# HKUST-Aerial-Robotics/FUEL

Measured on AMD Instinct MI355X. Metric: plan_cycles_per_sec, higher is better.
Workload: dtype u64 bit-planes / u16 (u32 beyond 255 voxels) exact squared distances / f32 ESDF / f64 log-odds and B-spline

## Files before the change

### fuel_amd/csrc/bspline.hip

```cpp
#include <cmath>
#include <cstring>
#include <vector>

#include "bspline_batch.h"

template <int CTRL, int ROW_MASK>
__device__ __forceinline__ double dpp_take(double v) {
  int lo = __double2loint(v), hi = __double2hiint(v);
  lo = __builtin_amdgcn_update_dpp(0, lo, CTRL, ROW_MASK, 0xF, false);
  hi = __builtin_amdgcn_update_dpp(0, hi, CTRL, ROW_MASK, 0xF, false);
  return __hiloint2double(hi, lo);
}
__device__ __forceinline__ double wave_sum(double v) {
  v += dpp_take<0xB1, 0xF>(v);
  v += dpp_take<0x4E, 0xF>(v);
  v += dpp_take<0x141, 0xF>(v);
  v += dpp_take<0x140, 0xF>(v);
  v += dpp_take<0x142, 0xA>(v);
  v += dpp_take<0x143, 0xC>(v);
  const int lo = __builtin_amdgcn_readlane(__double2loint(v), 63), hi = __builtin_amdgcn_readlane(__double2hiint(v), 63);
  return __hiloint2double(hi, lo);
}

__device__ __forceinline__ double dot3(const double* a, const double* b) {
  return a[0] * b[0] + a[1] * b[1] + a[2] * b[2];
}

#define EVAL_CONST 24
__device__ __forceinline__ double* eval_const(const BsplineArgs& A, unsigned char* smem_raw) {
  return reinterpret_cast<double*>(smem_raw) + 15 * (size_t)A.N;
}
__device__ void load_eval_const(const BsplineArgs& A, int c, unsigned char* smem_raw) {
  double* K = eval_const(A, smem_raw);
  const int l = threadIdx.x;
  if (l == 0) K[0] = A.pt_dist[c];
  if (l == 1) K[1] = A.knot_span ? A.knot_span[c] : 0.0;
  if (l == 2) K[2] = A.time_lb ? A.time_lb[c] : -1.0;
  if (l >= 3 && l < 12) K[l] = ((A.cost_function & FUELMI_COST_START) && A.start_state) ? A.start_state[(size_t)c * 9 + (l - 3)] : 0.0;
  if (l >= 12 && l < 21) K[l] = ((A.cost_function & FUELMI_COST_END) && A.end_state) ? A.end_state[(size_t)c * 9 + (l - 12)] : 0.0;
  __syncthreads();
}
template <int NWV>
__device__ double bspline_eval(const Geo& g, const float* __restrict__ dist, const BsplineArgs& A, int c,
                               const double* x, double* grad, unsigned char* smem_raw) {
  const double* K = eval_const(A, smem_raw);
  const int N = A.N, dim = A.dim;
  const int wv = NWV == 1 ? 0 : (int)(threadIdx.x >> 6);
  const bool is_sm = NWV == 1 || wv == 0, is_fe = NWV == 1 || wv == 1, is_di = NWV == 1 || wv == 2, is_mi = NWV == 1 || wv == 3;
  double* q = reinterpret_cast<double*>(smem_raw);
  double* tj = q + 3 * N;
  double* tv = tj + 3 * N;
  double* ta = tv + 3 * N;
  double* gw = ta + 3 * N;
  const int lane = threadIdx.x & 63;
  const bool opt_time = (A.cost_function & FUELMI_COST_MINTIME) != 0;
  const double dt = opt_time ? x[A.nvar - 1] : K[1];
  const double pt_dist = K[0];
  const fuelmi_bspline_cfg& P = A.cfg;

  for (int i = threadIdx.x; i < N; i += 64 * NWV)
    for (int j = 0; j < 3; ++j) q[3 * i + j] = (j < dim) ? x[dim * i + j] : 0.0;
  __syncthreads();

  double cost = 0.0, gt = 0.0;
  const double dt_inv = 1 / dt, dt_inv2 = dt_inv * dt_inv;
  const double pt_inv = 1 / pt_dist;
  const double r_2dt = 1 / (2 * dt), r_dt2 = 1 / (dt * dt), r_ndt2 = 1 / (-dt * dt), r_ndt3 = 1 / (-dt * dt * dt);
  DistGather G0;
  const bool gather0 = is_di && (A.cost_function & FUELMI_COST_DISTANCE) && lane < N;
  if (gather0) dist_gather_issue(g, dist, &q[3 * lane], G0);

  for (int i = lane; i < N; i += 64) {
    for (int k = 0; k < 3; ++k) {
      if (is_sm) tj[3 * i + k] = 0.0;
      if (is_fe) tv[3 * i + k] = 0.0;
      if (is_fe) ta[3 * i + k] = 0.0;
      if (is_mi) gw[3 * i + k] = 0.0;
    }
    if (is_sm && (A.cost_function & FUELMI_COST_SMOOTHNESS) && i + 3 < N) {
      double s = 0.0;
      for (int k = 0; k < 3; ++k) {
        double ji = (q[3 * (i + 3) + k] - 3 * q[3 * (i + 2) + k] + 3 * q[3 * (i + 1) + k] - q[3 * i + k]) * pt_inv;
        s += ji * ji;
        tj[3 * i + k] = 2 * ji * pt_inv;
      }
      cost += P.ld_smooth * s;
    }
    if (is_fe && (A.cost_function & FUELMI_COST_FEASIBILITY)) {
      if (i + 1 < N) {
        for (int k = 0; k < 3; ++k) {
          double vi = (q[3 * (i + 1) + k] - q[3 * i + k]) * dt_inv;
          double vd = fabs(vi) - P.max_vel;
          if (vd > 0.0) {
            cost += P.ld_feasi * (vd * vd);
            double sign = vi > 0 ? 1.0 : -1.0;
            double tmp = 2 * vd * sign * dt_inv;
            tv[3 * i + k] = tmp;
            if (opt_time) gt += P.ld_feasi * (tmp * (-vi));
          }
        }
      }
      if (i + 2 < N) {
        for (int k = 0; k < 3; ++k) {
          double ai = (q[3 * (i + 2) + k] - 2 * q[3 * (i + 1) + k] + q[3 * i + k]) * dt_inv2;
          double ad = fabs(ai) - P.max_acc;
          if (ad > 0.0) {
            cost += P.ld_feasi * (ad * ad);
            double sign = ai > 0 ? 1.0 : -1.0;
            double tmp = 2 * ad * sign * dt_inv2;
            ta[3 * i + k] = tmp;
            if (opt_time) gt += P.ld_feasi * (tmp * ai * (-2) * dt);
          }
        }
      }
    }
  }
  __syncthreads();
  if (is_mi && (A.cost_function & FUELMI_COST_WAYPOINTS) && lane == 0) {
    double s = 0.0;
    for (int w = 0; w < A.n_waypt; ++w) {
      const double* wp = A.waypoints + ((size_t)c * A.n_waypt + w) * 3;
      int idx = A.waypt_idx[(size_t)c * A.n_waypt + w];
      for (int k = 0; k < 3; ++k) {
        double dq = 1 / 6.0 * (q[3 * idx + k] + 4 * q[3 * (idx + 1) + k] + q[3 * (idx + 2) + k]) - wp[k];
        s += dq * dq;
        gw[3 * idx + k] += dq * (2.0 / 6.0);
        gw[3 * (idx + 1) + k] += dq * (8.0 / 6.0);
        gw[3 * (idx + 2) + k] += dq * (2.0 / 6.0);
      }
    }
    cost += P.ld_waypt * s;
  }
  __syncthreads();

  for (int i = lane; i < N; i += 64) {
    double gq[3] = {0.0, 0.0, 0.0};
    if (is_sm && (A.cost_function & FUELMI_COST_SMOOTHNESS)) {
      const double wgt[4] = {-1.0, 3.0, -3.0, 1.0};
      for (int s = 0; s < 4; ++s) {
        int j = i - s;
        if (j >= 0 && j + 3 < N)
          for (int k = 0; k < 3; ++k) gq[k] += P.ld_smooth * wgt[s] * tj[3 * j + k];
      }
    }
    if (is_di && (A.cost_function & FUELMI_COST_DISTANCE)) {
      double dg[3];
      double d = (i == lane && gather0) ? dist_gather_finish(g, G0, dg) : dist_with_grad_dev(g, dist, &q[3 * i], dg);
      double nrm = sqrt(dot3(dg, dg));
      if (nrm > 1e-4) {
        const double nrm_inv = 1 / nrm;
        for (int k = 0; k < 3; ++k) dg[k] *= nrm_inv;
      }
      if (d < P.dist0) {
        cost += P.ld_dist * ((d - P.dist0) * (d - P.dist0));
        for (int k = 0; k < 3; ++k) gq[k] += P.ld_dist * (2.0 * (d - P.dist0) * dg[k]);
      }
    }
    if (is_fe && (A.cost_function & FUELMI_COST_FEASIBILITY)) {
      for (int k = 0; k < 3; ++k) {
        double s = 0.0;
        if (i + 1 < N) s += -tv[3 * i + k];
        if (i >= 1) s += tv[3 * (i - 1) + k];
        if (i + 2 < N) s += ta[3 * i + k];
        if (i >= 1 && i + 1 < N) s += -2 * ta[3 * (i - 1) + k];
        if (i >= 2) s += ta[3 * (i - 2) + k];
        gq[k] += P.ld_feasi * s;
      }
    }
    {
      const bool is_start = is_mi && (A.cost_function & FUELMI_COST_START) && i < 3;
      const bool is_end = is_mi && (A.cost_function & FUELMI_COST_END) && i >= N - 3;
      for (int pass = 0; pass < 2; ++pass) {
        const bool as_end = (pass == 0) ? (!is_start && is_end) : (is_start && is_end);
        if (!(pass == 0 ? (is_start || is_end) : as_end)) continue;
        const int b0 = as_end ? N - 3 : 0, r = i - b0;
        const double* tgt = K + (as_end ? 12 : 3);
        const double w_pos = as_end ? 1.0 : 10.0, lam = as_end ? P.ld_end : P.ld_start;
        const bool have_vel = !as_end || A.end_n >= 2, have_acc = !as_end || A.end_n == 3;
        double c_b = 0.0, gt_b = 0.0;
        for (int k = 0; k < 3; ++k) {
          const double qa = q[3 * b0 + k], qb = q[3 * (b0 + 1) + k], qc = q[3 * (b0 + 2) + k];
          const double first = as_end ? qc : qa, last = as_end ? qa : qc;
          double dq = 1 / 6.0 * (first + 4 * qb + last) - tgt[k];
          c_b += w_pos * dq * dq;
          double gk = w_pos * 2 * dq * ((r == 1) ? (4 / 6.0) : (1 / 6.0));
          if (have_vel) {
            dq = r_2dt * (qc - qa) - tgt[3 + k];
            c_b += dq * dq;
            if (r == 0) gk += 2 * dq * (-1.0) * r_2dt;
            if (r == 2) gk += 2 * dq * 1.0 * r_2dt;
            gt_b += dq * (qc - qa) * r_ndt2;
          }
          if (have_acc) {
            dq = r_dt2 * (first - 2 * qb + last) - tgt[6 + k];
            c_b += dq * dq;
            gk += 2 * dq * ((r == 1) ? -2.0 : 1.0) * r_dt2;
            gt_b += dq * (first - 2 * qb + last) * r_ndt3;
          }
          gq[k] += lam * gk;
        }
        if (r == (as_end ? 2 : 0)) {
          cost += lam * c_b;
          if (opt_time) gt += lam * gt_b;
        }
      }
    }
    if (is_mi && (A.cost_function & FUELMI_COST_GUIDE) && i >= A.order && i < N - A.order) {
      const double* gp = A.guide_pts + ((size_t)c * A.n_guide + (i - A.order)) * 3;
      for (int k = 0; k < 3; ++k) {
        double d = q[3 * i + k] - gp[k];
        cost += P.ld_guide * d * d;
        gq[k] += P.ld_guide * 2 * d;
      }
    }
    if (is_mi && (A.cost_function & FUELMI_COST_WAYPOINTS))
      for (int k = 0; k < 3; ++k) gq[k] += P.ld_waypt * gw[3 * i + k];
    if (is_mi && (A.cost_function & FUELMI_COST_VIEWCONS) && i == A.view_idx[c]) {
      const double* p = A.view_pt + (size_t)c * 3;
      const double* dir = A.view_dir + (size_t)c * 3;
      double dn_ = sqrt(dot3(dir, dir));
      double v[3] = {dir[0] / dn_, dir[1] / dn_, dir[2] / dn_};
      double qp[3] = {q[3 * i] - p[0], q[3 * i + 1] - p[1], q[3 * i + 2] - p[2]};
      double pr = dot3(qp, v);
      double dn[3], dl[3];
      for (int k = 0; k < 3; ++k) {
        dn[k] = qp[k] - pr * v[k];
        dl[k] = pr * v[k];
      }
      double c_view = dot3(dn, dn);
      double vdn = dot3(v, dn);
      for (int k = 0; k < 3; ++k) gq[k] += P.ld_view * 2 * (dn[k] - vdn * v[k]);
      double norm_dl = sqrt(dot3(dl, dl));
      if (norm_dl < dn_) {
        c_view += P.wnl * (norm_dl - dn_) * (norm_dl - dn_);
        double vdl = dot3(v, dl);
        for (int k = 0; k < 3; ++k) gq[k] += P.ld_view * (P.wnl * 2 * (norm_dl - dn_) * (vdl * v[k]) / norm_dl);
      }
      cost += P.ld_view * c_view;
    }
    if (NWV == 1) {
      for (int j = 0; j < dim; ++j) grad[dim * i + j] = gq[j];
    } else {
      double* gpart = reinterpret_cast<double*>(smem_raw) + 15 * (size_t)N + EVAL_CONST + (size_t)wv * 3 * N;
      for (int j = 0; j < 3; ++j) gpart[3 * i + j] = gq[j];
    }
  }

  if (is_mi && (A.cost_function & FUELMI_COST_MINTIME) && lane == 0) {
    double duration = (N - A.order) * dt;
    double cst = duration, g_t = double(N - A.order);
    double lb = K[2];
    if (lb > 0 && duration < lb) {
      const double w_lb = 10;
      cst += w_lb * (duration - lb) * (duration - lb);
      g_t += w_lb * 2 * (duration - lb) * (N - A.order);
    }
    cost += P.ld_time * cst;
    gt += P.ld_time * g_t;
  }
  cost = wave_sum(cost);
  gt = wave_sum(gt);
  if (NWV == 1) {
    if (lane == 0 && opt_time) grad[A.nvar - 1] = gt;
    __syncthreads();
    return cost;
  }
  double* part = reinterpret_cast<double*>(smem_raw) + 15 * (size_t)N + EVAL_CONST;
  double* cpart = part + 12 * (size_t)N;
  if (lane == 0) cpart[wv] = cost, cpart[4 + wv] = gt;
  __syncthreads();
  for (int e = threadIdx.x; e < dim * N; e += 64 * NWV) {
    const int i = e / dim, j = e - i * dim;
    grad[e] = ((part[3 * i + j] + part[3 * N + 3 * i + j]) + part[6 * N + 3 * i + j]) + part[9 * N + 3 * i + j];
  }
  if (threadIdx.x == 0 && opt_time) grad[A.nvar - 1] = ((cpart[4] + cpart[5]) + cpart[6]) + cpart[7];
  const double total = ((cpart[0] + cpart[1]) + cpart[2]) + cpart[3];
  __syncthreads();
  return total;
}

__global__ void __launch_bounds__(256)
k_bspline_cost_grad(Geo g, const float* __restrict__ dist, BsplineArgs A) {
  extern __shared__ __attribute__((aligned(16))) unsigned char smem_raw[];
  const int c = blockIdx.x;
  load_eval_const(A, c, smem_raw);
  const double cost = bspline_eval<4>(g, dist, A, c, A.x + (size_t)c * A.nvar, A.grad + (size_t)c * A.nvar, smem_raw);
  if (threadIdx.x == 0) A.cost[c] = cost;
}

struct LbfgsArgs {
  int max_eval;
  unsigned long long max_ticks;
  double box_lo[3], box_hi[3];
  double* x_out;
  double* cost_out;
  int* evals_out;
};
#define LBFGS_MEM 8

__device__ __forceinline__ double wdot(const double* a, const double* b, int n) {
  double s = 0.0;
  for (int i = threadIdx.x; i < n; i += 64) s += a[i] * b[i];
  return wave_sum(s);
}

__global__ void __launch_bounds__(64)
k_bspline_optimize(Geo g, const float* __restrict__ dist, BsplineArgs A, LbfgsArgs L) {
  extern __shared__ __attribute__((aligned(16))) unsigned char smem_raw[];
  const int c = blockIdx.x, lane = threadIdx.x, n = A.nvar;
  double* w = reinterpret_cast<double*>(smem_raw) + 15 * (size_t)A.N + EVAL_CONST;
  load_eval_const(A, blockIdx.x, smem_raw);
  double *q = w, *gq = q + n, *xn = gq + n, *gn = xn + n, *d = gn + n, *best = d + n;
  double* S = best + n;
  double* Y = S + LBFGS_MEM * n;
  double* rho = Y + LBFGS_MEM * n;
  double* al = rho + LBFGS_MEM;
  const double* x0 = A.x + (size_t)c * n;
  const int npt = A.dim * A.N;
  auto lb_of = [&](int i, double q0) {
    if (A.dim == 1) return -1e300;
    if (i >= npt) return 0.0;
    return fmax(q0 - 10.0, L.box_lo[i % 3]);
  };
  auto ub_of = [&](int i, double q0) {
    if (A.dim == 1) return 1e300;
    if (i >= npt) return 5.0;
    return fmin(q0 + 10.0, L.box_hi[i % 3]);
  };
  for (int i = lane; i < n; i += 64) {
    double v = x0[i];
    if (A.dim != 1 && i < npt) v = fmax(fmin(v, L.box_hi[i % 3]), L.box_lo[i % 3]);
    q[i] = v;
    best[i] = v;
  }
  __syncthreads();
  auto start_val = [&](int i) {
    double v = x0[i];
    if (A.dim != 1 && i < npt) v = fmax(fmin(v, L.box_hi[i % 3]), L.box_lo[i % 3]);
    return v;
  };
  int evals = 0;
  const unsigned long long t_begin = wall_clock64();
  auto out_of_time = [&]() { return L.max_ticks != 0ull && wall_clock64() - t_begin > L.max_ticks; };
  double f = bspline_eval<1>(g, dist, A, c, q, gq, smem_raw);
  ++evals;
  double fbest = f;
  int hist = 0, head = 0;
  while (evals < L.max_eval && !out_of_time()) {
    for (int i = lane; i < n; i += 64) {
      const double sv = start_val(i), lo = lb_of(i, sv), hi = ub_of(i, sv);
      const bool at_lb = q[i] <= lo && gq[i] > 0, at_ub = q[i] >= hi && gq[i] < 0;
      d[i] = (at_lb || at_ub) ? 0.0 : -gq[i];
    }
    __syncthreads();
    for (int k = hist - 1; k >= 0; --k) {
      const int sl = (head + k) % LBFGS_MEM;
      const double a = wdot(S + sl * n, d, n) * rho[sl];
      if (lane == 0) al[sl] = a;
      for (int i = lane; i < n; i += 64) d[i] -= a * Y[sl * n + i];
      __syncthreads();
    }
    if (hist > 0) {
      const int sl = (head + hist - 1) % LBFGS_MEM;
      const double yy = wdot(Y + sl * n, Y + sl * n, n), sy = 1.0 / rho[sl];
      const double gamma = yy > 0 ? sy / yy : 1.0;
      for (int i = lane; i < n; i += 64) d[i] *= gamma;
      __syncthreads();
    }
    for (int k = 0; k < hist; ++k) {
      const int sl = (head + k) % LBFGS_MEM;
// ... 414 lines not shown
    }
    F.pt_dist[c] = s / double(n);
  }
}
static size_t fit_lds(int K, int degree) {
  const int n = K + degree - 1;
  return (size_t)(16 + 5 * n + 3 * n + 3 * n + 3 * (K + 4) + n + degree + 1) * sizeof(double);
}

__global__ __launch_bounds__(64) void k_bspline_boundary(int n, int p, const double* __restrict__ ts,
                                                         const double* __restrict__ ctrl, int ks, int ke,
                                                         double* __restrict__ start, double* __restrict__ end) {
  extern __shared__ __attribute__((aligned(16))) unsigned char smem_raw[];
  double* q = reinterpret_cast<double*>(smem_raw);
  double* u = q + 3 * n;
  const int c = blockIdx.x, lane = threadIdx.x;
  for (int i = lane; i < 3 * n; i += 64) q[i] = ctrl[(size_t)c * 3 * n + i];
  if (lane == 0) fit_uniform_knots(u, n, p, ts[c]);
  __syncthreads();
  if (lane <= ks) spline_boundary_value(q, n, p, u, lane, false, start + ((size_t)c * (ks + 1) + lane) * 3);
  else if (lane <= ks + 1 + ke)
    spline_boundary_value(q, n, p, u, lane - ks - 1, true, end + ((size_t)c * (ke + 1) + (lane - ks - 1)) * 3);
}

static int upload(fuelmi_bspline_dev* b, const void* src, size_t bytes, const void** dst) {
  *dst = nullptr;
  if (!src || bytes == 0) return FUELMI_OK;
  void* d = nullptr;
  HIPCHK(hipMalloc(&d, bytes));
  b->allocs.push_back(d);
  HIPCHK(hipMemcpyAsync(d, src, bytes, hipMemcpyHostToDevice, b->map->stream));
  *dst = d;
  return FUELMI_OK;
}

static void bspline_dev_orphan(void* p) { static_cast<fuelmi_bspline_dev*>(p)->map = nullptr; }
extern "C" void fuelmi_bspline_dev_destroy(fuelmi_bspline_dev* b) {
  if (!b) return;
  (void)hipSetDevice(b->device);
  if (b->map) {
    (void)hipStreamSynchronize(b->map->stream);
    std::lock_guard<std::mutex> lk(b->map->dep_mu);
    auto& deps = b->map->dependents;
    for (size_t k = 0; k < deps.size(); ++k)
      if (deps[k].obj == b) {
        deps.erase(deps.begin() + (long)k);
        break;
      }
  }
  for (void* p : b->allocs) (void)hipFree(p);
  for (DevScratch* sc : {&b->fit_in, &b->yaw_dev, &b->chk_dev, &b->smp_dev, &b->adj_dev}) sc->release();
  for (int k = 0; k < 2; ++k) {
    if (b->pin_out[k]) (void)hipHostFree(b->pin_out[k]);
    if (b->ev_out[k]) (void)hipEventDestroy(b->ev_out[k]);
  }
  delete b;
}

static int bspline_args_init(const fuelmi_bspline_cfg* cfg, const fuelmi_bspline_batch* in, BsplineArgs& A) {
  ARGCHK(in->dim >= 1 && in->dim <= 3 && in->point_num >= 4 && in->n_traj >= 1);
  ARGCHK(in->x && in->pt_dist);
  const int cf = in->cost_function;
  const bool opt_time = (cf & FUELMI_COST_MINTIME) != 0;
  ARGCHK(opt_time || in->knot_span);
  ARGCHK(!(cf & FUELMI_COST_START) || in->start_state);
  ARGCHK(!(cf & FUELMI_COST_END) || (in->end_state && in->end_n >= 1 && in->end_n <= 3));
  ARGCHK(!(cf & FUELMI_COST_GUIDE) || in->guide_pts);
  ARGCHK(!(cf & FUELMI_COST_WAYPOINTS) || (in->n_waypt >= 0 && (in->n_waypt == 0 || (in->waypoints && in->waypt_idx))));
  ARGCHK(!(cf & FUELMI_COST_VIEWCONS) || (in->view_pt && in->view_dir && in->view_idx));
  memset(&A, 0, sizeof(A));
  A.cfg = *cfg;
  A.cost_function = cf;
  A.dim = in->dim;
  A.N = in->point_num;
  A.C = in->n_traj;
  A.end_n = in->end_n;
  A.n_waypt = (cf & FUELMI_COST_WAYPOINTS) ? in->n_waypt : 0;
  A.nvar = opt_time ? A.dim * A.N + 1 : A.dim * A.N;
  A.order = (A.dim == 1) ? 3 : cfg->bspline_degree;
  A.n_guide = A.N - 2 * A.order;
  return FUELMI_OK;
}

extern "C" int fuelmi_bspline_dev_create(fuelmi_map* m, const fuelmi_bspline_cfg* cfg,
                                         const fuelmi_bspline_batch* in, fuelmi_bspline_dev** out) {
  ARGCHK(m && cfg && in && out);
  *out = nullptr;
  BsplineArgs A0;
  {
    const int rca = bspline_args_init(cfg, in, A0);
    if (rca) return rca;
  }
  const int cf = in->cost_function;
  const bool opt_time = (cf & FUELMI_COST_MINTIME) != 0;
  HIPCHK(hipSetDevice(m->device));
  fuelmi_bspline_dev* b = new fuelmi_bspline_dev;
  b->map = m;
  b->device = m->device;
  BsplineArgs& A = b->a;
  A = A0;
  (void)opt_time;
  b->lds = ((size_t)A.N * 3 * 5 + EVAL_CONST) * sizeof(double);
  b->lds_eval4 = b->lds + ((size_t)A.N * 12 + 8) * sizeof(double);
  if (b->lds_eval4 > 160 * 1024) {
    fuelmi_set_error("%d control points exceed the LDS budget", A.N);
    delete b;
    return FUELMI_ELIMIT;
  }
  const size_t C = (size_t)A.C;
  int rc = FUELMI_OK;
  auto up = [&](const void* src, size_t bytes, const void** dst) {
    if (rc == FUELMI_OK) rc = upload(b, src, bytes, dst);
  };
  up(in->x, C * A.nvar * sizeof(double), (const void**)&A.x);
  up(in->pt_dist, C * sizeof(double), (const void**)&A.pt_dist);
  up(in->knot_span, C * sizeof(double), (const void**)&A.knot_span);
  up(in->time_lb, C * sizeof(double), (const void**)&A.time_lb);
  if (cf & FUELMI_COST_START) up(in->start_state, C * 9 * sizeof(double), (const void**)&A.start_state);
  if (cf & FUELMI_COST_END) up(in->end_state, C * 9 * sizeof(double), (const void**)&A.end_state);
  if ((cf & FUELMI_COST_GUIDE) && A.n_guide > 0)
    up(in->guide_pts, C * A.n_guide * 3 * sizeof(double), (const void**)&A.guide_pts);
  if (A.n_waypt > 0) {
    up(in->waypoints, C * A.n_waypt * 3 * sizeof(double), (const void**)&A.waypoints);
    up(in->waypt_idx, C * A.n_waypt * sizeof(int), (const void**)&A.waypt_idx);
  }
  if (cf & FUELMI_COST_VIEWCONS) {
    up(in->view_pt, C * 3 * sizeof(double), (const void**)&A.view_pt);
    up(in->view_dir, C * 3 * sizeof(double), (const void**)&A.view_dir);
    up(in->view_idx, C * sizeof(int), (const void**)&A.view_idx);
  }
  if (rc == FUELMI_OK) {
    void* d = nullptr;
    if (hipMalloc(&d, C * sizeof(double)) == hipSuccess) {
      b->allocs.push_back(d);
      A.cost = (double*)d;
    } else
      rc = FUELMI_ENOMEM;
    if (rc == FUELMI_OK && hipMalloc(&d, C * A.nvar * sizeof(double)) == hipSuccess) {
      b->allocs.push_back(d);
      A.grad = (double*)d;
    } else
      rc = FUELMI_ENOMEM;
  }
  if (rc != FUELMI_OK) {
    fuelmi_bspline_dev_destroy(b);
    return rc;
  }
  if (b->lds_eval4 > 64 * 1024) {
    HIPCHK(hipFuncSetAttribute(reinterpret_cast<const void*>(&k_bspline_cost_grad),
                               hipFuncAttributeMaxDynamicSharedMemorySize, 160 * 1024));
  }
  {
    std::lock_guard<std::mutex> lk(m->dep_mu);
    m->dependents.push_back({b, &bspline_dev_orphan});
  }
  *out = b;
  return FUELMI_OK;
}

extern "C" int fuelmi_bspline_dev_eval(fuelmi_bspline_dev* b) {
  ARGCHK(b);
  HIPCHK(hipSetDevice(b->map->device));
  StageScope sc(b->map, FUELMI_K_BSPLINE);
  k_bspline_cost_grad<<<b->a.C, 256, b->lds_eval4, b->map->stream>>>(b->map->g, b->map->dist, b->a);
  HIPCHK(hipGetLastError());
  return FUELMI_OK;
}

extern "C" int fuelmi_bspline_dev_eval_pinned(fuelmi_bspline_dev* b, int slot) {
  ARGCHK(b && (slot == 0 || slot == 1));
  HIPCHK(hipSetDevice(b->map->device));
  const size_t C = (size_t)b->a.C, n = (size_t)b->a.nvar;
  if (!b->pin_out[slot]) {
    HIPCHK(hipHostMalloc(reinterpret_cast<void**>(&b->pin_out[slot]), (C + C * n) * sizeof(double), hipHostMallocDefault));
    HIPCHK(hipEventCreateWithFlags(&b->ev_out[slot], hipEventDisableTiming));
  }
  BsplineArgs A = b->a;
  A.cost = b->pin_out[slot];
  A.grad = b->pin_out[slot] + C;
  {
    StageScope sc(b->map, FUELMI_K_BSPLINE);
    k_bspline_cost_grad<<<A.C, 256, b->lds_eval4, b->map->stream>>>(b->map->g, b->map->dist, A);
    HIPCHK(hipGetLastError());
  }
  HIPCHK(hipEventRecord(b->ev_out[slot], b->map->stream));
  return FUELMI_OK;
}
extern "C" int fuelmi_bspline_dev_collect(fuelmi_bspline_dev* b, int slot, double* cost, double* grad) {
  ARGCHK(b && (slot == 0 || slot == 1) && cost && grad && b->pin_out[slot]);
  HIPCHK(hipSetDevice(b->map->device));
  HIPCHK(event_poll(b->ev_out[slot]));
  const size_t C = (size_t)b->a.C, n = (size_t)b->a.nvar;
  memcpy(cost, b->pin_out[slot], C * sizeof(double));
  memcpy(grad, b->pin_out[slot] + C, C * n * sizeof(double));
  return FUELMI_OK;
}

struct OptPlan {
  int npl, waves;
  size_t lds;
};
static int bspline_opt_plan(const BsplineArgs& A, OptPlan& p) {
  if (A.dim == 2) {
    fuelmi_set_error("the B-spline optimiser takes dim 1 or 3, not 2");
    return FUELMI_EINVAL;
  }
  const size_t n = (size_t)A.nvar;
  const size_t lds_eval = ((size_t)A.N * 3 * 5 + EVAL_CONST) * sizeof(double);
  p.npl = n <= 128 ? 2 : (n <= 256 ? 4 : 0);
  p.waves = (p.npl && A.C <= 256) ? 4 : 1;
  p.lds = p.npl ? lds_eval + ((size_t)A.N * 12 + 8) * sizeof(double) + 2 * n * sizeof(double)
                : lds_eval + ((6 + 2 * LBFGS_MEM) * n + 2 * LBFGS_MEM) * sizeof(double);
  if (p.lds > 160 * 1024) {
    fuelmi_set_error("%d variables exceed the LDS budget of the device optimiser", (int)n);
    return FUELMI_ELIMIT;
  }
  return FUELMI_OK;
}
static int bspline_opt_launch(const OptPlan& p, hipStream_t st, const Geo& g, const float* dist, const BsplineArgs& A,
                              const LbfgsArgs& L) {
  if (p.npl == 0 && p.lds > 64 * 1024)
    HIPCHK(hipFuncSetAttribute(reinterpret_cast<const void*>(&k_bspline_optimize),
                               hipFuncAttributeMaxDynamicSharedMemorySize, 160 * 1024));
  if (p.npl == 2 && p.waves == 4)
    k_bspline_optimize_r<2, 4><<<A.C, 256, p.lds, st>>>(g, dist, A, L);
  else if (p.npl == 4 && p.waves == 4)
    k_bspline_optimize_r<4, 4><<<A.C, 256, p.lds, st>>>(g, dist, A, L);
  else if (p.npl == 2)
    k_bspline_optimize_r<2, 1><<<A.C, 64, p.lds, st>>>(g, dist, A, L);
  else if (p.npl == 4)
    k_bspline_optimize_r<4, 1><<<A.C, 64, p.lds, st>>>(g, dist, A, L);
  else
    k_bspline_optimize<<<A.C, 64, p.lds, st>>>(g, dist, A, L);
  HIPCHK(hipGetLastError());
  return FUELMI_OK;
}

extern "C" int fuelmi_bspline_opt_plan(const fuelmi_bspline_batch* batch, int out3[3]) {
  ARGCHK(batch && out3);
  fuelmi_bspline_cfg cfg;
  memset(&cfg, 0, sizeof(cfg));
  cfg.bspline_degree = 3;
  BsplineArgs A;
  const int rca = bspline_args_init(&cfg, batch, A);
  if (rca) return rca;
  OptPlan p;
  const int rc = bspline_opt_plan(A, p);
  if (rc) return rc;
  out3[0] = p.npl, out3[1] = p.waves, out3[2] = (int)p.lds;
  return FUELMI_OK;
}

extern "C" int fuelmi_bspline_dev_optimize(fuelmi_bspline_dev* b, int max_eval, double* x_out, double* cost_out,
                                           int* evals_out) {
  return fuelmi_bspline_dev_optimize_timed(b, max_eval, -1.0, x_out, cost_out, evals_out);
}
extern "C" int fuelmi_bspline_dev_optimize_timed(fuelmi_bspline_dev* b, int max_eval, double max_time_s, double* x_out,
                                                 double* cost_out, int* evals_out) {
  ARGCHK(b && max_eval >= 1 && x_out && cost_out);
  fuelmi_map* m = b->map;
  HIPCHK(hipSetDevice(m->device));
  const BsplineArgs& A = b->a;
  const size_t C = (size_t)A.C, n = (size_t)A.nvar;
  OptPlan plan;
  {
    const int rcp = bspline_opt_plan(A, plan);
// ... 26 lines not shown
  }
  HIPCHK(hipMemcpyAsync(x_out, b->opt_x, C * n * sizeof(double), hipMemcpyDeviceToHost, m->stream));
  HIPCHK(hipMemcpyAsync(cost_out, b->opt_cost, C * sizeof(double), hipMemcpyDeviceToHost, m->stream));
  std::vector<int> ev(C);
  HIPCHK(hipMemcpyAsync(ev.data(), b->opt_evals, C * sizeof(int), hipMemcpyDeviceToHost, m->stream));
  HIPCHK(hipStreamSynchronize(m->stream));
  if (evals_out) memcpy(evals_out, ev.data(), C * sizeof(int));
  b->opt_valid = true;
  return FUELMI_OK;
}

extern "C" int fuelmi_bspline_dev_download(fuelmi_bspline_dev* b, double* cost, double* grad) {
  ARGCHK(b && cost && grad);
  HIPCHK(hipSetDevice(b->map->device));
  HIPCHK(hipMemcpyAsync(cost, b->a.cost, (size_t)b->a.C * sizeof(double), hipMemcpyDeviceToHost, b->map->stream));
  HIPCHK(hipMemcpyAsync(grad, b->a.grad, (size_t)b->a.C * b->a.nvar * sizeof(double), hipMemcpyDeviceToHost,
                        b->map->stream));
  HIPCHK(stream_wait(b->map->stream));
  return FUELMI_OK;
}

static int bspline_oneshot(fuelmi_map* m, const fuelmi_bspline_cfg* cfg, const fuelmi_bspline_batch* in, int max_eval,
                           double max_time_s, double* out_a, double* out_b, int* evals) {
  ARGCHK(m && cfg && in && out_a && out_b);
  BsplineArgs A;
  {
    const int rca = bspline_args_init(cfg, in, A);
    if (rca) return rca;
  }
  HIPCHK(hipSetDevice(m->device));
  const int cf = A.cost_function;
  const size_t C = (size_t)A.C, n = (size_t)A.nvar;
  struct Piece {
    const void* src;
    size_t bytes;
    const void** dst;
  };
  const Piece pieces[] = {
      {in->x, C * n * sizeof(double), (const void**)&A.x},
      {in->pt_dist, C * sizeof(double), (const void**)&A.pt_dist},
      {in->knot_span, in->knot_span ? C * sizeof(double) : 0, (const void**)&A.knot_span},
      {in->time_lb, in->time_lb ? C * sizeof(double) : 0, (const void**)&A.time_lb},
      {in->start_state, (cf & FUELMI_COST_START) ? C * 9 * sizeof(double) : 0, (const void**)&A.start_state},
      {in->end_state, (cf & FUELMI_COST_END) ? C * 9 * sizeof(double) : 0, (const void**)&A.end_state},
      {in->guide_pts, ((cf & FUELMI_COST_GUIDE) && A.n_guide > 0) ? C * A.n_guide * 3 * sizeof(double) : 0, (const void**)&A.guide_pts},
      {in->waypoints, A.n_waypt > 0 ? C * A.n_waypt * 3 * sizeof(double) : 0, (const void**)&A.waypoints},
      {in->waypt_idx, A.n_waypt > 0 ? C * A.n_waypt * sizeof(int) : 0, (const void**)&A.waypt_idx},
      {in->view_pt, (cf & FUELMI_COST_VIEWCONS) ? C * 3 * sizeof(double) : 0, (const void**)&A.view_pt},
      {in->view_dir, (cf & FUELMI_COST_VIEWCONS) ? C * 3 * sizeof(double) : 0, (const void**)&A.view_dir},
      {in->view_idx, (cf & FUELMI_COST_VIEWCONS) ? C * sizeof(int) : 0, (const void**)&A.view_idx},
  };
  size_t in_bytes = 0;
  for (const Piece& p : pieces) in_bytes += (p.bytes + 15) & ~(size_t)15;
  const size_t out_bytes = ((C * sizeof(double) + 15) & ~(size_t)15) + ((C * n * sizeof(double) + 15) & ~(size_t)15) +
                           ((C * sizeof(int) + 15) & ~(size_t)15);
  const size_t lds_eval = ((size_t)A.N * 3 * 5 + EVAL_CONST) * sizeof(double);
  OptPlan plan;
  if (max_eval > 0) {
    const int rcp = bspline_opt_plan(A, plan);
    if (rcp) return rcp;
  }
  QuerySlotGuard q;
  {
    const int rcq = q.acquire(m, in_bytes + out_bytes);
    if (rcq) return rcq;
  }
  unsigned char* at = q.s->pin;
  for (const Piece& p : pieces) {
    *p.dst = nullptr;
    if (!p.bytes || !p.src) continue;
    memcpy(at, p.src, p.bytes);
    *p.dst = at;
    at += (p.bytes + 15) & ~(size_t)15;
  }
  double* o_a = reinterpret_cast<double*>(q.s->pin + in_bytes);
  double* o_b = reinterpret_cast<double*>(q.s->pin + in_bytes + ((C * sizeof(double) + 15) & ~(size_t)15));
  int* o_e = reinterpret_cast<int*>(reinterpret_cast<unsigned char*>(o_b) + ((C * n * sizeof(double) + 15) & ~(size_t)15));
  if (max_eval <= 0) {
    const size_t lds4 = lds_eval + ((size_t)A.N * 12 + 8) * sizeof(double);
    if (lds4 > 160 * 1024) {
      fuelmi_set_error("%d control points exceed the LDS budget", A.N);
      return FUELMI_ELIMIT;
    }
    if (lds4 > 64 * 1024)
      HIPCHK(hipFuncSetAttribute(reinterpret_cast<const void*>(&k_bspline_cost_grad), hipFuncAttributeMaxDynamicSharedMemorySize,
                                 160 * 1024));
    A.cost = o_a, A.grad = o_b;
    k_bspline_cost_grad<<<A.C, 256, lds4, q.s->st>>>(m->g, m->dist, A);
  } else {
    LbfgsArgs L;
    L.max_eval = max_eval;
    L.max_ticks = max_time_s > 0.0 ? (unsigned long long)(max_time_s * 1e8) + 1ull : 0ull;
    for (int k = 0; k < 3; ++k) {
      L.box_lo[k] = m->cfg.box_min[k] + 0.1;
      L.box_hi[k] = m->cfg.box_max[k] - 0.1;
    }
    L.x_out = o_b, L.cost_out = o_a, L.evals_out = o_e;
    const int rcl = bspline_opt_launch(plan, q.s->st, m->g, m->dist, A, L);
    if (rcl) return rcl;
  }
  HIPCHK(hipGetLastError());
  HIPCHK(q.finish());
  memcpy(out_a, o_a, C * sizeof(double));
  memcpy(out_b, o_b, C * n * sizeof(double));
  if (evals && max_eval > 0) memcpy(evals, o_e, C * sizeof(int));
  return FUELMI_OK;
}

extern "C" int fuelmi_bspline_cost_grad(fuelmi_map* m, const fuelmi_bspline_cfg* cfg,
                                        const fuelmi_bspline_batch* batch, double* cost, double* grad) {
  ARGCHK(cost && grad);
  return bspline_oneshot(m, cfg, batch, 0, -1.0, cost, grad, nullptr);
}
extern "C" int fuelmi_bspline_optimize(fuelmi_map* m, const fuelmi_bspline_cfg* cfg, const fuelmi_bspline_batch* batch,
                                       int max_eval, double max_time_s, double* x_out, double* cost_out, int* evals_out) {
  ARGCHK(max_eval >= 1 && x_out && cost_out);
  return bspline_oneshot(m, cfg, batch, max_eval, max_time_s, cost_out, x_out, evals_out);
}

int fit_launch(fuelmi_map* m, const FitArgs& F, hipStream_t st) {
  const size_t lds = fit_lds(F.K, F.degree);
  if (lds > 160 * 1024) {
    fuelmi_set_error("%d samples exceed the LDS budget of the spline fit", F.K);
    return FUELMI_ELIMIT;
  }
  if (lds > 64 * 1024)
    HIPCHK(hipFuncSetAttribute(reinterpret_cast<const void*>(&k_bspline_fit), hipFuncAttributeMaxDynamicSharedMemorySize,
                               (int)lds));
  k_bspline_fit<<<F.C, 64, lds, st ? st : m->stream>>>(F);
  HIPCHK(hipGetLastError());
  return FUELMI_OK;
}

FitArgs fit_args(const fuelmi_bspline_dev* b, double* ts, double* points, double* derivs, int* skip) {
  const BsplineArgs& A = b->a;
  FitArgs F;
  memset(&F, 0, sizeof(F));
  F.C = A.C, F.K = A.N - A.cfg.bspline_degree + 1, F.degree = A.cfg.bspline_degree;
  F.ts = ts;
  F.points = points;
  F.derivs = derivs;
  F.ctrl = const_cast<double*>(A.x);
  F.stride = A.nvar;
  F.write_dt = (A.cost_function & FUELMI_COST_MINTIME) ? 1 : 0;
  F.knot_span = const_cast<double*>(A.knot_span);
  F.pt_dist = const_cast<double*>(A.pt_dist);
  F.start_state = const_cast<double*>(A.start_state);
  F.end_state = const_cast<double*>(A.end_state);
  F.skip = skip;
  return F;
}

SplineSrc opt_spline_src(const fuelmi_bspline_dev* b) {
  const BsplineArgs& A = b->a;
  const size_t nvar = (size_t)A.nvar;
  if (A.cost_function & FUELMI_COST_MINTIME) return {nullptr, A.N, b->opt_x, nvar, b->opt_x + (A.nvar - 1), nvar};
  return {nullptr, A.N, b->opt_x, nvar, A.knot_span, 1};
}

extern "C" int fuelmi_bspline_parameterize(fuelmi_map* m, int n_traj, int n_points, int degree, const double* ts,
                                           const double* points, const double* derivs, double* ctrl) {
  ARGCHK(m && ts && points && derivs && ctrl);
  ARGCHK(n_traj >= 1 && n_points >= 2 && degree >= 3 && degree <= 5);
  for (int c = 0; c < n_traj; ++c)
    if (!(ts[c] > 0)) {
      fuelmi_set_error("fuelmi_bspline_parameterize: time step of candidate %d is not positive", c);
      return FUELMI_EINVAL;
    }
  HIPCHK(hipSetDevice(m->device));
  const size_t C = (size_t)n_traj, K = (size_t)n_points, n = K + degree - 1;
  const size_t b_ts = C * sizeof(double), b_pts = C * K * 3 * sizeof(double), b_der = C * 12 * sizeof(double),
// ... 83 lines not shown
```

### fuel_amd/csrc/bspline_batch.h

```cpp
#ifndef FUELMI_BSPLINE_BATCH_H_
#define FUELMI_BSPLINE_BATCH_H_

#include <cmath>

#include "fuelmi_internal.h"
#include "spline_internal.h"

struct BsplineArgs {
  fuelmi_bspline_cfg cfg;
  int cost_function, dim, N, C, end_n, n_waypt, nvar, order, n_guide;
  const double* x;
  const double* pt_dist;
  const double* knot_span;
  const double* time_lb;
  const double* start_state;
  const double* end_state;
  const double* guide_pts;
  const double* waypoints;
  const int* waypt_idx;
  const double* view_pt;
  const double* view_dir;
  const int* view_idx;
  double* cost;
  double* grad;
};

struct fuelmi_bspline_dev {
  fuelmi_map* map;
  int device = 0;
  BsplineArgs a;
  std::vector<void*> allocs;
  size_t lds;
  size_t lds_eval4;
  double *opt_x = nullptr, *opt_cost = nullptr;
  int* opt_evals = nullptr;
  double* pin_out[2] = {nullptr, nullptr};
  hipEvent_t ev_out[2] = {nullptr, nullptr};
  bool opt_valid = false;
  DevScratch fit_in;
  DevScratch yaw_dev;
  DevScratch chk_dev;
  DevScratch smp_dev;
  DevScratch adj_dev;
};

struct FitArgs {
  int C, K, degree;
  const double* ts;
  const double* points;
  const double* derivs;
  double* ctrl;
  long stride;
  int write_dt;
  double* knot_span;
  double* pt_dist;
  double* start_state;
  double* end_state;
  const int* skip;
  const int* Ks;
  long pt_stride;
};

FitArgs fit_args(const fuelmi_bspline_dev* b, double* ts, double* points, double* derivs, int* skip);
int fit_launch(fuelmi_map* m, const FitArgs& F, hipStream_t st = nullptr);
SplineSrc opt_spline_src(const fuelmi_bspline_dev* b);

inline int spline_src_check(int n_prob, int degree, int max_ctrl, const int* n_ctrl, const double* pos_ctrl,
                            const double* knot_span, bool knots_given = false) {
  ARGCHK(n_ctrl && pos_ctrl && (knot_span || knots_given));
  for (int b = 0; b < n_prob; ++b) {
    ARGCHK(n_ctrl[b] >= degree + 1 && n_ctrl[b] <= max_ctrl);
    if (!knots_given) ARGCHK(std::isfinite(knot_span[b]) && knot_span[b] > 0.0);
    const double* P = pos_ctrl + (size_t)b * max_ctrl * 3;
    for (int k = 0; k < 3 * n_ctrl[b]; ++k) ARGCHK(std::fabs(P[k]) < 1e7);
  }
  return FUELMI_OK;
}
inline void spline_src_take(BlockLayout& L, size_t n, int max_ctrl, SplineSrc& s) {
  s.n_ctrl = L.take<int>(n), s.n_ctrl_all = 0;
  s.knot = L.take<double>(n), s.knot_stride = 1;
  s.pos = L.take<double>(n * max_ctrl * 3), s.pos_stride = (size_t)max_ctrl * 3;
}
inline int spline_src_upload(hipStream_t st, const SplineSrc& s, size_t n, int max_ctrl, const int* n_ctrl,
                             const double* pos_ctrl, const double* knot_span) {
  HIPCHK(hipMemcpyAsync(const_cast<int*>(s.n_ctrl), n_ctrl, n * sizeof(int), hipMemcpyHostToDevice, st));
  if (knot_span)
    HIPCHK(hipMemcpyAsync(const_cast<double*>(s.knot), knot_span, n * sizeof(double), hipMemcpyHostToDevice, st));
  else
    HIPCHK(hipMemsetAsync(const_cast<double*>(s.knot), 0, n * sizeof(double), st));
  HIPCHK(hipMemcpyAsync(const_cast<double*>(s.pos), pos_ctrl, n * max_ctrl * 3 * sizeof(double), hipMemcpyHostToDevice, st));
  return FUELMI_OK;
}

#endif
```

Measured before the change: 11290.

## Specialize B-spline cost kernel on cost mask and fold constant loads into prologue

The four-wave cost/gradient kernel is now templated on the cost-function mask, so common masks are compile-time constants and dead cost branches drop out. The separate constant-load phase and its barrier are merged into the control-point load, with dt and pt_dist read straight from global memory. When no waypoint term is present, the workgroup barriers around the waypoint phase become a wavefront-level fence. An environment-gated per-phase timing path is also added, which adds template instances and code size.

```diff
diff --git a/fuel_amd/csrc/bspline.hip b/fuel_amd/csrc/bspline.hip
--- a/fuel_amd/csrc/bspline.hip
+++ b/fuel_amd/csrc/bspline.hip
@@ -40,12 +40,26 @@
   if (l >= 12 && l < 21) K[l] = ((A.cost_function & FUELMI_COST_END) && A.end_state) ? A.end_state[(size_t)c * 9 + (l - 12)] : 0.0;
   __syncthreads();
 }
-template <int NWV>
+#define CF_RT (-1)
+__device__ __forceinline__ void wave_lds_order() {
+  __builtin_amdgcn_fence(__ATOMIC_RELEASE, "wavefront");
+  __builtin_amdgcn_wave_barrier();
+  __builtin_amdgcn_fence(__ATOMIC_ACQUIRE, "wavefront");
+}
+template <bool STAMP>
+__device__ __forceinline__ void phase_stamp(unsigned long long* stamp, int k, bool who) {
+  if constexpr (STAMP)
+    if (who) stamp[k] = wall_clock64();
+}
+template <int NWV, int CF = CF_RT, bool BATCH = false, bool STAMP = false>
 __device__ double bspline_eval(const Geo& g, const float* __restrict__ dist, const BsplineArgs& A, int c,
-                               const double* x, double* grad, unsigned char* smem_raw) {
-  const double* K = eval_const(A, smem_raw);
+                               const double* x, double* grad, unsigned char* smem_raw, unsigned long long* stamp = nullptr) {
+  static_assert(!BATCH || NWV == 4, "the batch form is the four-wave cost kernel's");
+  static_assert(!STAMP || NWV == 4, "stamps are the four-wave cost kernel's");
+  const int cf = CF == CF_RT ? A.cost_function : CF;
+  double* K = eval_const(A, smem_raw);
   const int N = A.N, dim = A.dim;
-  const int wv = NWV == 1 ? 0 : (int)(threadIdx.x >> 6);
+  const int wv = NWV == 1 ? 0 : (BATCH ? __builtin_amdgcn_readfirstlane((int)(threadIdx.x >> 6)) : (int)(threadIdx.x >> 6));
   const bool is_sm = NWV == 1 || wv == 0, is_fe = NWV == 1 || wv == 1, is_di = NWV == 1 || wv == 2, is_mi = NWV == 1 || wv == 3;
   double* q = reinterpret_cast<double*>(smem_raw);
   double* tj = q + 3 * N;
@@ -53,21 +67,46 @@
   double* ta = tv + 3 * N;
   double* gw = ta + 3 * N;
   const int lane = threadIdx.x & 63;
-  const bool opt_time = (A.cost_function & FUELMI_COST_MINTIME) != 0;
-  const double dt = opt_time ? x[A.nvar - 1] : K[1];
-  const double pt_dist = K[0];
+  const bool opt_time = (cf & FUELMI_COST_MINTIME) != 0;
   const fuelmi_bspline_cfg& P = A.cfg;
-
-  for (int i = threadIdx.x; i < N; i += 64 * NWV)
-    for (int j = 0; j < 3; ++j) q[3 * i + j] = (j < dim) ? x[dim * i + j] : 0.0;
-  __syncthreads();
+  double dt, pt_dist;
+  if constexpr (!BATCH) {
+    dt = opt_time ? x[A.nvar - 1] : K[1];
+    pt_dist = K[0];
+    for (int i = threadIdx.x; i < N; i += 64 * NWV)
+      for (int j = 0; j < 3; ++j) q[3 * i + j] = (j < dim) ? x[dim * i + j] : 0.0;
+    __syncthreads();
+  } else {
+    auto q_src = [&](int e) {
+      if (dim == 3) return x[e];
+      const int i = e / 3, j = e - 3 * i;
+      return (j < dim) ? x[dim * i + j] : 0.0;
+    };
+    const int e0 = threadIdx.x;
+    const double q0 = e0 < 3 * N ? q_src(e0) : 0.0;
+    dt = opt_time ? x[A.nvar - 1] : (A.knot_span ? A.knot_span[c] : 0.0);
+    pt_dist = A.pt_dist[c];
+    double kv = 0.0;
+    if (is_mi) {
+      const double* src = nullptr;
+      if (lane == 2 && A.time_lb) src = A.time_lb + c;
+      if (lane >= 3 && lane < 12 && (cf & FUELMI_COST_START) && A.start_state) src = A.start_state + (size_t)c * 9 + (lane - 3);
+      if (lane >= 12 && lane < 21 && (cf & FUELMI_COST_END) && A.end_state) src = A.end_state + (size_t)c * 9 + (lane - 12);
+      kv = src ? *src : (lane == 2 ? -1.0 : 0.0);
+    }
+    if (is_mi && lane >= 2 && lane < 21) K[lane] = kv;
+    if (e0 < 3 * N) q[e0] = q0;
+    for (int e = e0 + 64 * NWV; e < 3 * N; e += 64 * NWV) q[e] = q_src(e);
+    __syncthreads();
+  }
+  phase_stamp<STAMP>(stamp, 1, threadIdx.x == 0);
 
   double cost = 0.0, gt = 0.0;
   const double dt_inv = 1 / dt, dt_inv2 = dt_inv * dt_inv;
   const double pt_inv = 1 / pt_dist;
   const double r_2dt = 1 / (2 * dt), r_dt2 = 1 / (dt * dt), r_ndt2 = 1 / (-dt * dt), r_ndt3 = 1 / (-dt * dt * dt);
   DistGather G0;
-  const bool gather0 = is_di && (A.cost_function & FUELMI_COST_DISTANCE) && lane < N;
+  const bool gather0 = is_di && (cf & FUELMI_COST_DISTANCE) && lane < N;
   if (gather0) dist_gather_issue(g, dist, &q[3 * lane], G0);
 
   for (int i = lane; i < N; i += 64) {
@@ -77,7 +116,7 @@
       if (is_fe) ta[3 * i + k] = 0.0;
       if (is_mi) gw[3 * i + k] = 0.0;
     }
-    if (is_sm && (A.cost_function & FUELMI_COST_SMOOTHNESS) && i + 3 < N) {
+    if (is_sm && (cf & FUELMI_COST_SMOOTHNESS) && i + 3 < N) {
       double s = 0.0;
       for (int k = 0; k < 3; ++k) {
         double ji = (q[3 * (i + 3) + k] - 3 * q[3 * (i + 2) + k] + 3 * q[3 * (i + 1) + k] - q[3 * i + k]) * pt_inv;
@@ -86,7 +125,7 @@
       }
       cost += P.ld_smooth * s;
     }
-    if (is_fe && (A.cost_function & FUELMI_COST_FEASIBILITY)) {
+    if (is_fe && (cf & FUELMI_COST_FEASIBILITY)) {
       if (i + 1 < N) {
         for (int k = 0; k < 3; ++k) {
           double vi = (q[3 * (i + 1) + k] - q[3 * i + k]) * dt_inv;
@@ -115,8 +154,9 @@
       }
     }
   }
-  __syncthreads();
-  if (is_mi && (A.cost_function & FUELMI_COST_WAYPOINTS) && lane == 0) {
+  const bool wg_barriers = !BATCH || (cf & FUELMI_COST_WAYPOINTS);
+  if (wg_barriers) __syncthreads(); else wave_lds_order();
+  if (is_mi && (cf & FUELMI_COST_WAYPOINTS) && lane == 0) {
     double s = 0.0;
     for (int w = 0; w < A.n_waypt; ++w) {
       const double* wp = A.waypoints + ((size_t)c * A.n_waypt + w) * 3;
@@ -131,11 +171,11 @@
     }
     cost += P.ld_waypt * s;
   }
-  __syncthreads();
+  if (wg_barriers) __syncthreads();
 
   for (int i = lane; i < N; i += 64) {
     double gq[3] = {0.0, 0.0, 0.0};
-    if (is_sm && (A.cost_function & FUELMI_COST_SMOOTHNESS)) {
+    if (is_sm && (cf & FUELMI_COST_SMOOTHNESS)) {
       const double wgt[4] = {-1.0, 3.0, -3.0, 1.0};
       for (int s = 0; s < 4; ++s) {
         int j = i - s;
@@ -143,9 +183,13 @@
           for (int k = 0; k < 3; ++k) gq[k] += P.ld_smooth * wgt[s] * tj[3 * j + k];
       }
     }
-    if (is_di && (A.cost_function & FUELMI_COST_DISTANCE)) {
+    if (is_di && (cf & FUELMI_COST_DISTANCE)) {
       double dg[3];
       double d = (i == lane && gather0) ? dist_gather_finish(g, G0, dg) : dist_with_grad_dev(g, dist, &q[3 * i], dg);
+      if constexpr (STAMP) {
+        asm volatile("" : "+v"(d));
+        phase_stamp<STAMP>(stamp, 2, i == 0);
+      }
       double nrm = sqrt(dot3(dg, dg));
       if (nrm > 1e-4) {
         const double nrm_inv = 1 / nrm;
@@ -156,7 +200,7 @@
         for (int k = 0; k < 3; ++k) gq[k] += P.ld_dist * (2.0 * (d - P.dist0) * dg[k]);
       }
     }
-    if (is_fe && (A.cost_function & FUELMI_COST_FEASIBILITY)) {
+    if (is_fe && (cf & FUELMI_COST_FEASIBILITY)) {
       for (int k = 0; k < 3; ++k) {
         double s = 0.0;
         if (i + 1 < N) s += -tv[3 * i + k];
@@ -168,8 +212,8 @@
       }
     }
     {
-      const bool is_start = is_mi && (A.cost_function & FUELMI_COST_START) && i < 3;
-      const bool is_end = is_mi && (A.cost_function & FUELMI_COST_END) && i >= N - 3;
+      const bool is_start = is_mi && (cf & FUELMI_COST_START) && i < 3;
+      const bool is_end = is_mi && (cf & FUELMI_COST_END) && i >= N - 3;
       for (int pass = 0; pass < 2; ++pass) {
         const bool as_end = (pass == 0) ? (!is_start && is_end) : (is_start && is_end);
         if (!(pass == 0 ? (is_start || is_end) : as_end)) continue;
@@ -205,7 +249,7 @@
         }
       }
     }
-    if (is_mi && (A.cost_function & FUELMI_COST_GUIDE) && i >= A.order && i < N - A.order) {
+    if (is_mi && (cf & FUELMI_COST_GUIDE) && i >= A.order && i < N - A.order) {
       const double* gp = A.guide_pts + ((size_t)c * A.n_guide + (i - A.order)) * 3;
       for (int k = 0; k < 3; ++k) {
         double d = q[3 * i + k] - gp[k];
@@ -213,9 +257,9 @@
         gq[k] += P.ld_guide * 2 * d;
       }
     }
-    if (is_mi && (A.cost_function & FUELMI_COST_WAYPOINTS))
+    if (is_mi && (cf & FUELMI_COST_WAYPOINTS))
       for (int k = 0; k < 3; ++k) gq[k] += P.ld_waypt * gw[3 * i + k];
-    if (is_mi && (A.cost_function & FUELMI_COST_VIEWCONS) && i == A.view_idx[c]) {
+    if (is_mi && (cf & FUELMI_COST_VIEWCONS) && i == A.view_idx[c]) {
       const double* p = A.view_pt + (size_t)c * 3;
       const double* dir = A.view_dir + (size_t)c * 3;
       double dn_ = sqrt(dot3(dir, dir));
@@ -246,7 +290,7 @@
     }
   }
 
-  if (is_mi && (A.cost_function & FUELMI_COST_MINTIME) && lane == 0) {
+  if (is_mi && (cf & FUELMI_COST_MINTIME) && lane == 0) {
     double duration = (N - A.order) * dt;
     double cst = duration, g_t = double(N - A.order);
     double lb = K[2];
@@ -269,6 +313,7 @@
   double* cpart = part + 12 * (size_t)N;
   if (lane == 0) cpart[wv] = cost, cpart[4 + wv] = gt;
   __syncthreads();
+  phase_stamp<STAMP>(stamp, 3, threadIdx.x == 0);
   for (int e = threadIdx.x; e < dim * N; e += 64 * NWV) {
     const int i = e / dim, j = e - i * dim;
     grad[e] = ((part[3 * i + j] + part[3 * N + 3 * i + j]) + part[6 * N + 3 * i + j]) + part[9 * N + 3 * i + j];
@@ -279,13 +324,21 @@
   return total;
 }
 
+template <int CF, bool STAMP>
 __global__ void __launch_bounds__(256)
-k_bspline_cost_grad(Geo g, const float* __restrict__ dist, BsplineArgs A) {
+k_bspline_cost_grad(Geo g, const float* __restrict__ dist, BsplineArgs A, unsigned long long* stamps) {
   extern __shared__ __attribute__((aligned(16))) unsigned char smem_raw[];
   const int c = blockIdx.x;
-  load_eval_const(A, c, smem_raw);
-  const double cost = bspline_eval<4>(g, dist, A, c, A.x + (size_t)c * A.nvar, A.grad + (size_t)c * A.nvar, smem_raw);
+  unsigned long long* stamp = STAMP ? stamps + 8 * (size_t)c : nullptr;
+  phase_stamp<STAMP>(stamp, 0, threadIdx.x == 0);
+  const double cost = bspline_eval<4, CF, true, STAMP>(g, dist, A, c, A.x + (size_t)c * A.nvar, A.grad + (size_t)c * A.nvar,
+                                                       smem_raw, stamp);
   if (threadIdx.x == 0) A.cost[c] = cost;
+  if constexpr (STAMP) {
+    __builtin_amdgcn_s_waitcnt(0);
+    __syncthreads();
+    phase_stamp<STAMP>(stamp, 4, threadIdx.x == 0);
+  }
 }
 
 struct LbfgsArgs {
@@ -866,6 +919,67 @@
   return FUELMI_OK;
 }
 
+#define CF_NORMAL (FUELMI_COST_SMOOTHNESS | FUELMI_COST_DISTANCE | FUELMI_COST_FEASIBILITY | FUELMI_COST_START | FUELMI_COST_END)
+#define CF_GUIDE (FUELMI_COST_SMOOTHNESS | FUELMI_COST_GUIDE | FUELMI_COST_START | FUELMI_COST_END)
+#define CF_YAW (FUELMI_COST_SMOOTHNESS | FUELMI_COST_WAYPOINTS | FUELMI_COST_START | FUELMI_COST_END)
+template <bool STAMP>
+static CostKernel cost_kernel_of(int cf) {
+  switch (cf) {
+    case CF_NORMAL: return &k_bspline_cost_grad<CF_NORMAL, STAMP>;
+    case CF_NORMAL | FUELMI_COST_MINTIME: return &k_bspline_cost_grad<CF_NORMAL | FUELMI_COST_MINTIME, STAMP>;
+    case CF_GUIDE: return &k_bspline_cost_grad<CF_GUIDE, STAMP>;
+    case CF_YAW: return &k_bspline_cost_grad<CF_YAW, STAMP>;
+    default: return &k_bspline_cost_grad<CF_RT, STAMP>;
+  }
+}
+static int cost_kernel_lds(CostKernel k, size_t lds) {
+  if (lds > 64 * 1024)
+    HIPCHK(hipFuncSetAttribute(reinterpret_cast<const void*>(k), hipFuncAttributeMaxDynamicSharedMemorySize, 160 * 1024));
+  return FUELMI_OK;
+}
+static int cost_launch_timed(hipStream_t st, const Geo& g, const float* dist, const BsplineArgs& A, size_t lds) {
+  const CostKernel k = cost_kernel_of<true>(A.cost_function);
+  const int rca = cost_kernel_lds(k, lds);
+  if (rca) return rca;
+  unsigned long long* dbg = nullptr;
+  const size_t n = (size_t)A.C * 8;
+  HIPCHK(hipMalloc(reinterpret_cast<void**>(&dbg), n * sizeof(unsigned long long)));
+  HIPCHK(hipMemsetAsync(dbg, 0, n * sizeof(unsigned long long), st));
+  k<<<A.C, 256, lds, st>>>(g, dist, A, dbg);
+  HIPCHK(hipGetLastError());
+  HIPCHK(hipStreamSynchronize(st));
+  std::vector<unsigned long long> d(n);
+  HIPCHK(hipMemcpy(d.data(), dbg, n * sizeof(unsigned long long), hipMemcpyDeviceToHost));
+  HIPCHK(hipFree(dbg));
+  static const char* const name[4] = {"prologue", "gathers", "pass2", "store"};
+  double sum[5] = {0, 0, 0, 0, 0}, worst[5] = {0, 0, 0, 0, 0};
+  unsigned long long t0 = ~0ull, t1 = 0;
+  for (int w = 0; w < A.C; ++w) {
+    const unsigned long long* r = &d[(size_t)w * 8];
+    const unsigned long long at[5] = {r[0], r[1], r[2] ? r[2] : r[1], r[3], r[4]};
+    for (int p = 0; p < 5; ++p) {
+      const double us = p < 4 ? (double)(at[p + 1] - at[p]) / 100.0 : (double)(at[4] - at[0]) / 100.0;
+      sum[p] += us, worst[p] = std::max(worst[p], us);
+    }
+    t0 = std::min(t0, r[0]), t1 = std::max(t1, r[4]);
+  }
+  char line[512];
+  int o = std::snprintf(line, sizeof line, "[bsp-timing] mask 0x%x N %d C %d us avg/max:", A.cost_function, A.N, A.C);
+  for (int p = 0; p < 4; ++p)
+    o += std::snprintf(line + o, sizeof line - o, " %s %.3f/%.2f", name[p], sum[p] / A.C, worst[p]);
+  std::snprintf(line + o, sizeof line - o, " | workgroup %.3f/%.2f | first start to last end %.2f", sum[4] / A.C, worst[4],
+                (double)(t1 - t0) / 100.0);
+  std::fprintf(stderr, "%s\n", line);
+  return FUELMI_OK;
+}
+static int cost_launch(CostKernel k, hipStream_t st, const Geo& g, const float* dist, const BsplineArgs& A, size_t lds) {
+  static const bool timing = getenv("FUELMI_BSP_TIMING") != nullptr;
+  if (timing) return cost_launch_timed(st, g, dist, A, lds);
+  k<<<A.C, 256, lds, st>>>(g, dist, A, nullptr);
+  HIPCHK(hipGetLastError());
+  return FUELMI_OK;
+}
+
 extern "C" int fuelmi_bspline_dev_create(fuelmi_map* m, const fuelmi_bspline_cfg* cfg,
                                          const fuelmi_bspline_batch* in, fuelmi_bspline_dev** out) {
   ARGCHK(m && cfg && in && out);
@@ -930,9 +1044,13 @@
     fuelmi_bspline_dev_destroy(b);
     return rc;
   }
-  if (b->lds_eval4 > 64 * 1024) {
-    HIPCHK(hipFuncSetAttribute(reinterpret_cast<const void*>(&k_bspline_cost_grad),
-                               hipFuncAttributeMaxDynamicSharedMemorySize, 160 * 1024));
+  b->eval_kern = cost_kernel_of<false>(A.cost_function);
+  {
+    const int rck = cost_kernel_lds(b->eval_kern, b->lds_eval4);
+    if (rck) {
+      fuelmi_bspline_dev_destroy(b);
+      return rck;
+    }
   }
   {
     std::lock_guard<std::mutex> lk(m->dep_mu);
@@ -946,9 +1064,7 @@
   ARGCHK(b);
   HIPCHK(hipSetDevice(b->map->device));
   StageScope sc(b->map, FUELMI_K_BSPLINE);
-  k_bspline_cost_grad<<<b->a.C, 256, b->lds_eval4, b->map->stream>>>(b->map->g, b->map->dist, b->a);
-  HIPCHK(hipGetLastError());
-  return FUELMI_OK;
+  return cost_launch(b->eval_kern, b->map->stream, b->map->g, b->map->dist, b->a, b->lds_eval4);
 }
 
 extern "C" int fuelmi_bspline_dev_eval_pinned(fuelmi_bspline_dev* b, int slot) {
@@ -964,8 +1080,8 @@
   A.grad = b->pin_out[slot] + C;
   {
     StageScope sc(b->map, FUELMI_K_BSPLINE);
-    k_bspline_cost_grad<<<A.C, 256, b->lds_eval4, b->map->stream>>>(b->map->g, b->map->dist, A);
-    HIPCHK(hipGetLastError());
+    const int rcl = cost_launch(b->eval_kern, b->map->stream, b->map->g, b->map->dist, A, b->lds_eval4);
+    if (rcl) return rcl;
   }
   HIPCHK(hipEventRecord(b->ev_out[slot], b->map->stream));
   return FUELMI_OK;
@@ -1158,11 +1274,14 @@
       fuelmi_set_error("%d control points exceed the LDS budget", A.N);
       return FUELMI_ELIMIT;
     }
-    if (lds4 > 64 * 1024)
-      HIPCHK(hipFuncSetAttribute(reinterpret_cast<const void*>(&k_bspline_cost_grad), hipFuncAttributeMaxDynamicSharedMemorySize,
-                                 160 * 1024));
+    const CostKernel kern = cost_kernel_of<false>(A.cost_function);
+    {
+      const int rck = cost_kernel_lds(kern, lds4);
+      if (rck) return rck;
+    }
     A.cost = o_a, A.grad = o_b;
-    k_bspline_cost_grad<<<A.C, 256, lds4, q.s->st>>>(m->g, m->dist, A);
+    const int rcl = cost_launch(kern, q.s->st, m->g, m->dist, A, lds4);
+    if (rcl) return rcl;
   } else {
     LbfgsArgs L;
     L.max_eval = max_eval;
diff --git a/fuel_amd/csrc/bspline_batch.h b/fuel_amd/csrc/bspline_batch.h
--- a/fuel_amd/csrc/bspline_batch.h
+++ b/fuel_amd/csrc/bspline_batch.h
@@ -25,10 +25,13 @@
   double* grad;
 };
 
+typedef void (*CostKernel)(Geo, const float*, BsplineArgs, unsigned long long*);
+
 struct fuelmi_bspline_dev {
   fuelmi_map* map;
   int device = 0;
   BsplineArgs a;
+  CostKernel eval_kern = nullptr;
   std::vector<void*> allocs;
   size_t lds;
   size_t lds_eval4;
```

Result: slower. 11060 (-2.1%).
